# paritybit-ai/XFL

Measured on AMD Instinct MI355X. Metric: 2048-bit Paillier encrypts/s (device-resident), higher is better.
Workload: dtype u32; 1 GPU; DJN private-key (CRT) encrypt, obfuscated, precision 7, 1000000 float64 plaintexts/GPU resident in HBM; key_bits=2048, elements_per_gpu=1000000, fixed_base_window_bits=23, fixed_base_window_split=False, parallelism=shard1, table_bytes=193273528320

## Files before the change

### __graft_entry__.py

```python
import os
import sys

ROOT = os.path.dirname(os.path.abspath(__file__))
if ROOT not in sys.path:
    sys.path.insert(0, ROOT)


def build() -> None:
    from xfl_amd import build as b
    b.build()
    from oracle import build as ob
    ob.build()
    import runpy
    for script in ("build.py", "build_redc_block.py"):
        try:
            runpy.run_path(os.path.join(ROOT, "tests", "native", script), run_name="tests_native_build")["build"]()
        except Exception as exc:
            print(f"warning: device self-test harnesses not built ({script}): {exc}", file=sys.stderr)
    import xfl_amd
    from xfl_amd import _native
    _native.lib()


def smoke() -> None:
    import numpy as np

    from oracle import paillier_oracle as O
    from xfl_amd import _native as nat
    from xfl_amd.paillier.utils import getprimeover
    import random
    import math

    rng = random.Random(7)
    while True:
        p, q = getprimeover(1024, rng=rng), getprimeover(1024, rng=rng)
        if p != q and math.gcd(p - 1, q - 1) == 2:
            break
    n = p * q
    x = rng.getrandbits(n.bit_length()) | (1 << (n.bit_length() - 1))
    h = pow(-(x * x), n, n * n)
    dk = nat.DeviceKey(2048, n, p, q, h, device=0)
    ok = O.derive_private(p, q, h)
    vals = np.random.default_rng(0).standard_normal(64) * 10
    ms = [O.encode_element(ok, float(v), 7)[0] for v in vals]
    rs = [rng.randrange(1, ok["djn_exp_bound"]) for _ in vals]
    ct = nat.words_to_ints(dk.encrypt_words(nat.ints_to_words(ms, dk.nw), nat.ints_to_words(rs, dk.rand_words)))
    want = [O.encrypt_m(ok, m, r) for m, r in zip(ms, rs)]
# ... 11 lines not shown
```

### xfl_amd/csrc/bn_dev.hpp

```cpp
#pragma once
#include <hip/hip_runtime.h>
#include <stdint.h>

namespace xhe {

#define XHE_DEV __device__ __forceinline__
#define XHE_INL __attribute__((always_inline))

#ifndef XHE_SQ_ACC
#define XHE_SQ_ACC 2
#endif
XHE_DEV uint64_t mad64(uint32_t a, uint32_t b, uint64_t c) {
  asm("v_mad_u64_u32 %0, vcc, %1, %2, %0" : "+v"(c) : "v"(a), "v"(b) : "vcc");
  return c;
}
template <int N>
XHE_DEV void mad_shift(uint64_t (&T)[N], const uint32_t (&b)[N], uint32_t a) {
  int j = 1;
#pragma unroll
  for (; j + 6 <= N; j += 6)
    asm("v_mad_u64_u32 %0, vcc, %7, %8, %1\n\t"
        "v_mad_u64_u32 %1, vcc, %7, %9, %2\n\t"
        "v_mad_u64_u32 %2, vcc, %7, %10, %3\n\t"
        "v_mad_u64_u32 %3, vcc, %7, %11, %4\n\t"
// ... 473 lines not shown
    sq_columns<0, HI>(b, lo, 0ull, q, hi);
    uint64_t T[L];
#pragma unroll
    for (int j = 0; j < L; ++j) T[j] = lo[j];
    hi.sync();
    red_rows(T, hi);
    normalize(T, b);
  }
  template <class HI>
  XHE_DEV void red_rows(uint64_t (&T)[L], const HI& hi) const {
    const uint32_t* Np = np();
    NRes R;
    load_res(Np, R);
    uint64_t x0 = T[0];
    uint32_t m = ((uint32_t)x0 * n0inv) & MASK;
    uint4 cur = hi.load4(0);
    int i = 0;
    for (; i + 4 <= S; i += 4) {
      uint4 nxt = hi.load4(i + 4 < S4 ? i + 4 : i);
      __builtin_amdgcn_sched_barrier(0);
      step1_red(Np, R, T, cur.x, m, x0);
      __builtin_amdgcn_sched_barrier(0);
      step1_red(Np, R, T, cur.y, m, x0);
      __builtin_amdgcn_sched_barrier(0);
      step1_red(Np, R, T, cur.z, m, x0);
      __builtin_amdgcn_sched_barrier(0);
      step1_red(Np, R, T, cur.w, m, x0);
      __builtin_amdgcn_sched_barrier(0);
      cur = nxt;
    }
#pragma unroll
    for (int r = 0; r < (S & 3); ++r) step1_red(Np, R, T, comp4(cur, r), m, x0);
  }

  XHE_DEV void step(const uint32_t* Np, uint64_t (&T)[L], const uint32_t (&b)[L], uint32_t ai, uint32_t ai_next,
                    uint32_t& m, uint64_t& x0, bool lead) const {
    static_assert(L >= 5, "pipelined step needs L >= 5");
    uint64_t xn = 0;
    uint32_t t = 0, mn = 0;
    int stage = 0;
    auto advance = [&]() XHE_INL {
      if (stage == 0) {
        T[0] += x0 >> W;
        asm volatile("" : "+v"(T[0]));
      } else if (stage == 1) {
        xn = mad64(ai_next, b[0], T[0]);
        asm volatile("" : "+v"(xn));
      } else if (stage == 2) {
        t = (uint32_t)xn * n0inv;
        asm volatile("" : "+v"(t));
      } else if (stage == 3) {
        mn = G::bcast0(t & MASK);
        asm volatile("" : "+v"(mn));
      }
      ++stage;
      __builtin_amdgcn_sched_barrier(0);
    };
    x0 = madN(Np, m, 0, x0);
    mac4(Np, T, b, ai, m, 1);
    advance();
    int j = 5;
#pragma unroll
    for (; j + 8 <= L; j += 8) {
      mac8(Np, T, b, ai, m, j);
      if (stage < 4) advance();
    }
// ... 328 lines not shown
```

### xfl_amd/csrc/keyconst.hpp

```cpp
#pragma once
#include <algorithm>
#include <cstdint>
#include <stdexcept>
#include <utility>
#include <vector>

#include "hostbn.hpp"
#include "keydev.hpp"
#include "rns_layout.hpp"

namespace xhe {

struct ModSpec {
  int S, W;
  int S4() const { return (S + 3) & ~3; }
  BigU R() const { return pow2((size_t)W * S); }
};

struct KeySpec {
  int K;
  bool priv, djn;
  ModSpec mp2, mp2L, mp2X;
  ModSpec mp;
  ModSpec mn2, mn2X;
// ... 256 lines not shown
    }
    put(rows, {m, &ModDev::Rpow});
  }

  KeyDev bind(const uint32_t* base) const {
    KeyDev r = kd;
    for (const Binding& b : binds) {
      const uint32_t* p = base + b.off;
      if (b.dst.w) r.*b.dst.w = p;
      else if (b.dst.d) r.*b.dst.d = reinterpret_cast<const uint2*>(p);
      else (r.*b.dst.m).*b.dst.mw = p;
    }
    return r;
  }

 private:
  struct Binding {
    Dst dst;
    size_t off;
  };
  std::vector<Binding> binds;
};

namespace pq {
constexpr ModF m2[2] = {&KeyDev::p2, &KeyDev::q2}, m2L[2] = {&KeyDev::p2L, &KeyDev::q2L},
               m2X[2] = {&KeyDev::p2X, &KeyDev::q2X}, m1[2] = {&KeyDev::p, &KeyDev::q},
               dm[2] = {&KeyDev::dp, &KeyDev::dq};
constexpr RowF nprime[2] = {&KeyDev::p2_nprime, &KeyDev::q2_nprime}, rns[2] = {&KeyDev::rns_p, &KeyDev::rns_q},
               nR2[2] = {&KeyDev::nR2_p2, &KeyDev::nR2_q2}, nR2L[2] = {&KeyDev::nR2_p2L, &KeyDev::nR2_q2L},
               nR[2] = {&KeyDev::nR_p2, &KeyDev::nR_q2}, R1C[2] = {&KeyDev::R1C_p2X, &KeyDev::R1C_q2X},
               nR2C[2] = {&KeyDev::nR2C_p2X, &KeyDev::nR2C_q2X}, m1_words[2] = {&KeyDev::pm1_words, &KeyDev::qm1_words},
               inv_lim[2] = {&KeyDev::pinv_lim, &KeyDev::qinv_lim}, hR[2] = {&KeyDev::hpR, &KeyDev::hqR},
               topc[2] = {&KeyDev::topc_p, &KeyDev::topc_q}, mu[2] = {&KeyDev::mu_p, &KeyDev::mu_q},
               e_words[2] = {&KeyDev::ep_words, &KeyDev::eq_words},
               x_kn2[2] = {&KeyDev::x_kn2_p, &KeyDev::x_kn2_q}, x_rmn[2] = {&KeyDev::x_rmn_p, &KeyDev::x_rmn_q},
               x_topc[2] = {&KeyDev::x_topc_p, &KeyDev::x_topc_q}, x_fold[2] = {&KeyDev::x_fold_p, &KeyDev::x_fold_q},
               x_hpR[2] = {&KeyDev::x_hpR_p, &KeyDev::x_hpR_q};
constexpr PairF x_dwt[2] = {&KeyDev::x_dwt_p, &KeyDev::x_dwt_q}, x_dw[2] = {&KeyDev::x_dw_p, &KeyDev::x_dw_q};
constexpr IntF m1_bits[2] = {&KeyDev::pm1_bits, &KeyDev::qm1_bits}, e_bits[2] = {&KeyDev::ep_bits, &KeyDev::eq_bits};
}

struct Prime {
  BigU X, Y, X2, n, h;
};

struct DigitMod {
  const BigU& M;
  ModSpec s;
  BigU R, RM, Rinv;
  DigitMod(const BigU& M_, const ModSpec& s_) : M(M_), s(s_), R(s_.R()), RM(mod(R, M_)), Rinv(modinv(RM, M_)) {}
};

inline std::vector<uint32_t> digit_pairs(const DigitMod& d, const BigU& Xw) {
  const BigU e = mulmod(mod(Xw, d.M), d.Rinv, d.M);
  BigU Q;
  divmod(add(Xw, mul(d.R, sub(d.M, e))), d.M, &Q, nullptr);
  const BigU f = submod(mod(Q, d.M), d.RM, d.M);
  const std::vector<uint32_t> el = e.to_limbs(d.s.W, d.s.S), fl = f.to_limbs(d.s.W, d.s.S);
  std::vector<uint32_t> v(2 * (size_t)d.s.S);
  for (int i = 0; i < d.s.S; ++i) {
    v[2 * i] = el[i];
    v[2 * i + 1] = fl[i];
  }
  return v;
}

// ... 88 lines not shown
    im.put_limbs(mulmod(pr[i].n, mulmod(CR, RxP, X2), X2), sx, pq::nR2C[i]);
  }
}

inline void decrypt_constants(KeyImage& im, const KeySpec& s, const BigU& n, Prime (&pr)[2]) {
  const ModSpec& s1 = s.mp;
  const BigU T = s1.R();
  for (int i = 0; i < 2; ++i) im.put_mod(pr[i].X, s1, pq::m1[i]);
  for (int i = 0; i < 2; ++i) {
    const BigU m1 = sub(pr[i].X, BigU(1));
    im.kd.*pq::m1_bits[i] = (int)m1.bits();
    im.put_words(m1, s.nw() / 2 + 1, pq::m1_words[i]);
  }
  for (int i = 0; i < 2; ++i) im.put_limbs(modinv(pr[i].X, T), s1, pq::inv_lim[i]);
  BigU Tm[2];
  for (int i = 0; i < 2; ++i) {
    const BigU& X = pr[i].X;
    const BigU x = mod(add(BigU(1), mul(sub(X, BigU(1)), n)), pr[i].X2);
    BigU L;
    divmod(sub(x, BigU(1)), X, &L, nullptr);
    pr[i].h = modinv(L, X);
    Tm[i] = mod(T, X);
  }
  for (int i = 0; i < 2; ++i) im.put_limbs(mulmod(pr[i].h, Tm[i], pr[i].X), s1, pq::hR[i]);
  im.put_limbs(mulmod(modinv(pr[1].X, pr[0].X), Tm[0], pr[0].X), s1, &KeyDev::qinvpR);
  im.put_limbs(pr[1].X, s1, &KeyDev::q_lim);
  if (s.K == 2048)
    for (int i = 0; i < 2; ++i) im.put(mask_plus_e(pr[i].X, mod(s.pmd.R(), pr[i].X), s.pmd), pq::topc[i]);
  if (s.K == 2048 && s.djn)
    for (int i = 0; i < 2; ++i) {
      const BigU &X = pr[i].X, RX = mod(s.pmd.R(), X), R2 = mulmod(RX, RX, X);
      im.put_limbs(mulmod(mod(pr[i].Y, X), mulmod(R2, R2, X), X), s.pmd, pq::mu[i]);
    }
}

inline void pdigit_constants(KeyImage& im, const KeySpec& s, const Prime& pr, int i) {
  const BigU &X = pr.X, &X2 = pr.X2;
  const DigitMod d(X, s.pd);
  digit_modulus(im, d, X2, pq::dm[i], pq::x_kn2[i], pq::x_rmn[i]);
  im.put(mask_plus_e(X, d.RM, d.s), pq::x_topc[i]);
  im.put_limbs(mulmod(mod(pr.Y, X), mulmod(mulmod(d.RM, d.RM, X), d.RM, X), X), d.s, pq::x_fold[i]);
  const BigU Rx2 = mod(d.R, X2), R2 = mulmod(Rx2, Rx2, X2), R4 = mulmod(R2, R2, X2);
  im.put(digit_pairs(d, mulmod(R4, modinv(mod(s.mp2.R(), X2), X2), X2)), pq::x_dwt[i]);
  im.put(digit_pairs(d, R4), pq::x_dw[i]);
  im.put_limbs(mulmod(pr.h, d.RM, X), d.s, pq::x_hpR[i]);
}

inline void exponent_constants(KeyImage& im, const KeySpec& s, const BigU& n, const Prime (&pr)[2]) {
  im.put_limbs(shl(pr[0].X, 1), s.mp, &KeyDev::p2x_lim);
  im.put_limbs(pr[0].X, s.mp, &KeyDev::p_lim);
  for (int i = 0; i < 2; ++i) {
    const BigU e = mod(n, mul(pr[i].X, sub(pr[i].X, BigU(1))));
    im.kd.*pq::e_bits[i] = (int)e.bits();
    im.put_words(e, s.nw(), pq::e_words[i]);
  }
}

inline std::vector<uint32_t> inverse_base_limbs(const ModSpec& s, const BigU& h, const BigU& P) {
  std::vector<uint32_t> v = mulmod(modinv(mod(h, P), P), mod(s.R(), P), P).to_limbs(s.W, s.S);
  v.resize((size_t)s.S4(), 0u);
  return v;
}

inline KeyImage derive_key_constants(const KeySpec& s, const BigU& n, const BigU* p, const BigU* q, const BigU* h) {
  KeyImage im;
  KeyDev& kd = im.kd;
// ... 35 lines not shown
```

### xfl_amd/csrc/keydev.hpp

```cpp
#pragma once
#include <cstdint>

#include <hip/hip_vector_types.h>

namespace xhe {

struct ModDev {
  const uint32_t* N;
  const uint32_t* R1;
  const uint32_t* R2;
  const uint32_t* R3;
  uint32_t n0inv;
  const uint32_t* Rpow;
};

constexpr int kRawChunk = 32;
constexpr int kRpowRows = kRawChunk + 2;

struct KeyDev {
  int K, nw, n2w;
  int priv, djn;
  const uint32_t* n_words;
  const uint32_t* n2_words;
  const uint32_t* maxpos;
// ... 8 lines not shown
  ModDev p2, q2;
  ModDev p2L, q2L;
  ModDev p2X, q2X;
  ModDev n2X;
  const uint32_t* nR2_p2;
  const uint32_t *nR_p2, *nR_q2;
  const uint32_t *nR2C_p2X, *nR2C_q2X;
  const uint32_t *R1C_p2X, *R1C_q2X;
  const uint32_t* nR2_q2;
  const uint32_t* nR2_p2L;
  const uint32_t* nR2_q2L;
  const uint32_t* q2invR_p2;
  const uint32_t* q2_lim;
  const uint32_t* p2x4_lim;
  const uint32_t* tab_p2;
  const uint32_t* tab_q2;
  int64_t tab_rs;
  int win, nwin, nhi;
  ModDev p, q;
  const uint32_t* pm1_words;
  const uint32_t* qm1_words;
  int pm1_bits, qm1_bits;
  const uint32_t* pinv_lim;
  const uint32_t* qinv_lim;
  const uint32_t* hpR;
  const uint32_t* hqR;
  const uint32_t* qinvpR;
  const uint32_t* q_lim;
  const uint32_t* p2x_lim;
  const uint32_t* p_lim;
  int pmd;
  const uint32_t *topc_p, *topc_q;
  const uint32_t *mu_p, *mu_q;
  int ndig;
  ModDev nd;
  const uint32_t *nd_kn2, *nd_rmn, *nd_topc;
  const uint2 *nd_dw, *nd_d1;
  const uint2* nd_dwt;
  int pub_nd;
  int pmdx;
  ModDev dp, dq;
  const uint32_t *x_kn2_p, *x_kn2_q, *x_rmn_p, *x_rmn_q, *x_topc_p, *x_topc_q, *x_fold_p, *x_fold_q;
  const uint2 *x_dwt_p, *x_dwt_q;
  int pmdx_dec;
  const uint2 *x_dw_p, *x_dw_q;
  const uint32_t *x_hpR_p, *x_hpR_q;
  const uint32_t *p2_nprime, *q2_nprime;
  const uint32_t *rns, *rns_p, *rns_q;
  const uint32_t *n2w_N, *n2w_np, *n2w_C, *n2w_R2;
  const uint32_t* n2_mu;
  ModDev nL;
  const uint32_t* n2_limL;
};

}
```

### xfl_amd/csrc/pdigit_dev.hpp

```cpp
#pragma once
#include "bn_dev.hpp"

namespace xhe {

struct PmdLdsQ {
  const uint32_t* q;
  XHE_DEV uint4 load4(int i) const { return *reinterpret_cast<const uint4*>(q + (i >> 2) * 256); }
};

template <int K_>
struct PMD {
  static constexpr int K = K_, W = 28, BL = 6;
  static constexpr int NQ = (2 * K + 3) / 4;
  static constexpr uint32_t MASK = (1u << W) - 1u;
  static_assert((K - 1) % BL == 0, "positions 1..K-1 in blocks of 6");
  static_assert((double)(3 * K + 2) * (double)(1ull << 57) < 18446744073709551616.0, "accumulator bound");

  uint32_t p[K];
  uint32_t n0inv;

  XHE_DEV void init(const uint32_t* __restrict__ P, uint32_t ninv) {
#pragma unroll
    for (int j = 0; j < K; ++j) p[j] = __builtin_amdgcn_readfirstlane(P[j]);
    n0inv = ninv;
// ... 348 lines not shown
    constexpr int LQ = (LW + 3) / 4;
    constexpr int NW = HW < LW ? HW : LW;
    static_assert(HW >= 8 && HW <= 4 * LQ, "at least one block of the chain, at most a whole sum");
    uint32_t s[4 * LQ];
#pragma unroll
    for (int q = 0; q < LQ; ++q) {
      const uint4 v = *reinterpret_cast<const uint4*>(slot + (EQ + q) * 256);
      s[4 * q] = v.x, s[4 * q + 1] = v.y, s[4 * q + 2] = v.z, s[4 * q + 3] = v.w;
    }
    uint64_t cy;
    add8<true>(s, lam, 0, cy);
#pragma unroll
    for (int k = 8; k + 8 <= NW; k += 8) add8<false>(s, lam, k, cy);
#pragma unroll
    for (int k = NW & ~7; k < NW; ++k)
      asm("v_addc_co_u32_e64 %0, %1, %0, %2, %1" : "+v"(s[k]), "+s"(cy) : "v"(lam[k]));
#pragma unroll
    for (int k = NW; k < LW; ++k) asm("v_addc_co_u32_e64 %0, %1, 0, %0, %1" : "+v"(s[k]), "+s"(cy));
#pragma unroll
    for (int q = 0; q < LQ; ++q)
      *reinterpret_cast<uint4*>(slot + (EQ + q) * 256) = make_uint4(s[4 * q], s[4 * q + 1], s[4 * q + 2], s[4 * q + 3]);
  }
  XHE_DEV static void lam_add_slot(uint32_t* slot, const uint32_t* other) {
    constexpr int LQ = (LW + 3) / 4;
    uint32_t o[4 * LQ];
#pragma unroll
    for (int q = 0; q < LQ; ++q) {
      const uint4 v = *reinterpret_cast<const uint4*>(other + (EQ + q) * 256);
      o[4 * q] = v.x, o[4 * q + 1] = v.y, o[4 * q + 2] = v.z, o[4 * q + 3] = v.w;
    }
    lam_add<4 * LQ>(slot, o);
  }

  XHE_DEV void finish(const uint32_t (&a)[K], uint32_t (&c)[K], uint32_t* slot, const uint32_t* Pl) const {
    constexpr int LQ = (LW + 3) / 4;
    {
      uint32_t s[4 * LQ + 1];
#pragma unroll
      for (int q = 0; q < LQ; ++q) {
        const uint4 v = *reinterpret_cast<const uint4*>(slot + (EQ + q) * 256);
        s[4 * q] = v.x, s[4 * q + 1] = v.y, s[4 * q + 2] = v.z, s[4 * q + 3] = v.w;
      }
      s[4 * LQ] = 0u;
      auto limb = [&](int i) -> uint32_t {
        const int bit = W * i, k = bit >> 5, sh = bit & 31;
        return i < K ? (__builtin_amdgcn_alignbit(k + 1 < LW ? s[k + 1] : 0u, s[k], sh) & MASK) : 0u;
      };
#pragma unroll
      for (int q = 0; q < EQ; ++q)
        *reinterpret_cast<uint4*>(slot + q * 256) = make_uint4(limb(4 * q), limb(4 * q + 1), limb(4 * q + 2), limb(4 * q + 3));
    }
    __builtin_amdgcn_sched_barrier(0);
    uint32_t t[K];
#pragma unroll
    for (int j = 0; j < K; ++j) t[j] = a[j];
    Mont<K, W, 1> MN;
    MN.init(Pl, n0inv);
    MN.mul(t, PmdLdsQ{slot});
    uint32_t cy = 0;
#pragma unroll
    for (int j = 0; j < K; ++j) {
      const uint32_t x = c[j] + t[j] + cy;
      c[j] = j + 1 < K ? (x & MASK) : x;
      cy = j + 1 < K ? (x >> W) : 0u;
    }
  }

  XHE_DEV static void normalize(const uint64_t (&T)[K], uint32_t (&b)[K]) {
    uint64_t cy = 0;
#pragma unroll
    for (int j = 0; j < K; ++j) {
      const uint64_t x = T[j] + cy;
      b[j] = j + 1 < K ? ((uint32_t)x & MASK) : (uint32_t)x;
      cy = x >> W;
      __builtin_amdgcn_sched_barrier(0);
    }
  }

  XHE_DEV void to_mont2(const uint32_t (&a)[K], const uint32_t (&c)[K], uint32_t (&x)[2 * K]) const {
    uint64_t T[2 * K];
#pragma unroll
    for (int j = 0; j < K; ++j) {
      T[j] = 0;
      T[K + j] = a[j];
    }
#pragma unroll
    for (int i = 0; i < K; ++i) {
#pragma unroll
      for (int j = 0; j < K; ++j) T[i + j] = mad64s(c[j], p[i], T[i + j]);
    }
    uint64_t cy = 0;
#pragma unroll
    for (int j = 0; j < 2 * K; ++j) {
      const uint64_t v = T[j] + cy;
      x[j] = j + 1 < 2 * K ? ((uint32_t)v & MASK) : (uint32_t)v;
      cy = v >> W;
    }
  }
// ... 13 lines not shown
#pragma unroll
    for (int j = 1; j < K; ++j) T[i + j] = mad64s(mi, M.p[j], T[i + j]);
    __builtin_amdgcn_sched_barrier(0);
  }
#pragma unroll
  for (int j = 0; j < K; ++j) {
    const uint64_t x = T[K + j] + cy;
    t[j] = j + 1 < K ? ((uint32_t)x & MASK) : (uint32_t)x;
    cy = x >> 28;
  }
}

template <int K>
XHE_DEV void pmd_redc_words(const Mont<K, 28, 1>& MN, uint32_t* slot, const uint32_t* __restrict__ mw, int nw,
                            uint32_t (&t)[K]) {
  constexpr uint32_t MASK = PMD<K>::MASK;
  auto limb = [&](int j) -> uint32_t {
    const int bit = 28 * j, k = bit >> 5, sh = bit & 31;
    const uint32_t lo = word_or0(mw, k, nw);
    const uint32_t hi = sh + 28 > 32 ? word_or0(mw, k + 1, nw) : 0u;
    return j < 2 * K ? (uint32_t)((((uint64_t)hi << 32) | lo) >> sh) & MASK : 0u;
  };
#pragma unroll
  for (int q = 0; q < PMD<K>::EQ; ++q)
    *reinterpret_cast<uint4*>(slot + q * 256) =
        make_uint4(limb(K + 4 * q), limb(K + 4 * q + 1), limb(K + 4 * q + 2), limb(K + 4 * q + 3));
#pragma unroll
  for (int j = 0; j < K; ++j) t[j] = limb(j);
  __builtin_amdgcn_sched_barrier(0);
  MN.redc_wide(t, PmdLdsQ{slot});
}

template <int K>
XHE_DEV void pmd_lam_plain(const PMD<K>& M, uint32_t* slot, const uint32_t* __restrict__ mw, int nw,
                           const uint32_t* mu, const uint32_t* Pl) {
  using D = PMD<K>;
  constexpr int LQ = (D::LW + 3) / 4;
  Mont<K, 28, 1> MN;
  MN.init(Pl, M.n0inv);
  uint32_t t[K];
  pmd_redc_words<K>(MN, slot, mw, nw, t);
  __builtin_amdgcn_sched_barrier(0);
  MN.mul(t, ARow{mu});
  uint32_t s[4 * LQ];
#pragma unroll
  for (int k = 0; k < 4 * LQ; ++k) {
    const int bit = 32 * k, j = bit / 28, sh = bit - 28 * j;
    uint64_t v = j < K ? (uint64_t)t[j] : 0ull;
    if (j + 1 < K) v |= (uint64_t)t[j + 1] << 28;
    if (j + 2 < K) v |= (uint64_t)t[j + 2] << 56;
    s[k] = k < D::LW ? (uint32_t)(v >> sh) : 0u;
  }
#pragma unroll
  for (int q = 0; q < LQ; ++q)
    *reinterpret_cast<uint4*>(slot + (D::EQ + q) * 256) = make_uint4(s[4 * q], s[4 * q + 1], s[4 * q + 2], s[4 * q + 3]);
}

template <int K>
XHE_DEV uint32_t pmd_sub(uint32_t (&r)[K], const uint32_t (&s)[K]) {
  int64_t br = 0;
#pragma unroll
  for (int j = 0; j < K; ++j) {
    const int64_t v = (int64_t)r[j] - (int64_t)s[j] + br;
    r[j] = (uint32_t)v & ((1u << 28) - 1u);
    br = v >> 28;
  }
  return br ? 1u : 0u;
}

template <int K>
XHE_DEV bool pmd_csub(const PMD<K>& M, uint32_t (&r)[K]) {
  int64_t br = 0;
#pragma unroll
  for (int j = 0; j < K; ++j) br = ((int64_t)r[j] - (int64_t)M.p[j] + br) >> 28;
  const bool ge = br == 0;
  br = 0;
#pragma unroll
  for (int j = 0; j < K; ++j) {
    const int64_t v = (int64_t)r[j] - (int64_t)(ge ? M.p[j] : 0u) + br;
    r[j] = (uint32_t)v & ((1u << 28) - 1u);
    br = v >> 28;
  }
  return ge;
}

template <int K>
XHE_DEV void pmd_mod_small(const PMD<K>& M, uint32_t (&m)[K]) {
  constexpr uint32_t MASK = PMD<K>::MASK;
  const uint32_t mt = (m[K - 1] << 4) | (m[K - 2] >> 24);
  const uint32_t pt = (M.p[K - 1] << 4) | (M.p[K - 2] >> 24);
  const uint32_t q = mt / (pt + 1u);
  uint64_t cy = 0;
  int64_t br = 0;
#pragma unroll
  for (int j = 0; j < K; ++j) {
    const uint64_t qp = (uint64_t)q * M.p[j] + cy;
    cy = qp >> 28;
    const int64_t v = (int64_t)m[j] - (int64_t)(qp & MASK) + br;
    m[j] = (uint32_t)v & MASK;
    br = v >> 28;
  }
#pragma unroll
  for (int t = 0; t < 3; ++t) pmd_csub<K>(M, m);
}

template <int K>
XHE_DEV void pmd_from_mont2(const PMD<K>& M, const uint32_t (&X)[2 * K], const uint32_t* RmodP, uint32_t (&e)[K],
                            uint32_t (&f)[K]) {
  uint32_t m[K];
  {
    uint64_t T[2 * K];
#pragma unroll
    for (int j = 0; j < 2 * K; ++j) T[j] = X[j];
    pmd_redc_wide<K>(M, T, e, m);
  }
  __builtin_amdgcn_sched_barrier(0);
  const bool ge = pmd_csub<K>(M, e);
  __builtin_amdgcn_sched_barrier(0);
  pmd_mod_small<K>(M, m);
  __builtin_amdgcn_sched_barrier(0);
  int64_t br = 0;
#pragma unroll
  for (int j = 0; j < K; ++j) {
    const int64_t v = (int64_t)(ge ? RmodP[j] : 0u) - (int64_t)m[j] + br;
    f[j] = (uint32_t)v & ((1u << 28) - 1u);
    br = v >> 28;
  }
  if (br) {
    int64_t cy = 0;
#pragma unroll
    for (int j = 0; j < K; ++j) {
      const int64_t v = (int64_t)f[j] + (int64_t)M.p[j] + cy;
      f[j] = (uint32_t)v & ((1u << 28) - 1u);
      cy = v >> 28;
    }
  }
// ... 650 lines not shown
```

### xfl_amd/csrc/xhe.hip

```cpp
#include <hip/hip_runtime.h>
#include <stdint.h>
#include <stdlib.h>
#include <string.h>

#include <chrono>
#include <cmath>
#include <cstdio>
#include <memory>
#include <mutex>
#include <atomic>
#include <stdexcept>
#include <unordered_map>
#include <utility>
#include <string>
#include <type_traits>
#include <vector>

#include "../../include/xhe.h"
#include "abi_common.hpp"
#include "hostbn.hpp"
#include "keyconst.hpp"
#include "paths.hpp"
#include "xhe_kernels.hpp"
#include "fermat_dev.hpp"
// ... 545 lines not shown
    if (!on) return;
    if (hipEventRecord(b, s) != hipSuccess) return;
    std::lock_guard<std::mutex> lk(g_prof_mu);
    g_prof.push_back({name, a, b});
  }
};

template <class Sh, class MP2 = typename Sh::MP2>
void crt_enc_launch(const xhe_key* k, int64_t n, uint32_t* ws, uint32_t* ct, hipStream_t s) {
  const int blocks = (int)((n * MP2::TPI + 255) / 256);
  if constexpr (MP2::TPI == 1)
    launch((k_crt_enc_w<MP2, 2 * Sh::K / 32>), dim3(blocks), dim3(256), s, k->kd, k->kd.p2.N, n, ws, ct);
  else
    launch(k_crt_enc<MP2>, dim3(blocks), dim3(256), s, k->kd, k->kd.p2.N, n, ws, ct);
}

template <class Sh>
void encrypt_impl(const xhe_key* k, const uint32_t* m, const uint32_t* r, int64_t count, uint32_t* ct, hipStream_t s) {
  using MP2 = typename Sh::MP2;
  int64_t chunk = std::min<int64_t>(count, kChunk);
  WsScope wsc(s);
  uint32_t* ws = wsc.get<uint32_t>((size_t)2 * 2 * MP2::S4 * chunk * sizeof(uint32_t));
  uint2* xst = nullptr;
  uint32_t *xrows = nullptr, *xwords = nullptr;
  for (int64_t off = 0; off < count; off += chunk) {
    int64_t n = std::min(chunk, count - off);
    switch (paths::enc_djn(Sh::K, MP2::TPI, k->kd.pmd, k->kd.pmdx, n, pins())) {
      case paths::EncDjn::PMD:
        if constexpr (Sh::K == 2048) {
          ProfScope ps("k_djn_pmd", s);
          const int G = paths::pmd_split(n, pins());
          const dim3 grid((unsigned)((n * G + 127) / 128), 2);
          auto run = [&](auto kern) {
            launch(kern, grid, dim3(128), s, k->kd, k->kd.p.N, k->kd.q.N, k->kd.p2.N, k->kd.q2.N,
                   m + (size_t)off * k->nw, r + (size_t)off * k->rand_words, k->rand_words, n, ws);
          };
          if (G == 16) run(k_djn_pmd<MP2, 37, Sh::RW, 16>);
          else if (G == 4) run(k_djn_pmd<MP2, 37, Sh::RW, 4>);
          else run(k_djn_pmd<MP2, 37, Sh::RW, 1>);
          crt_enc_launch<Sh>(k, n, ws, ct + (size_t)off * k->n2w, s);
          continue;
        } else no_path("encrypt (k_djn_pmd)");
      case paths::EncDjn::PMDX:
        if constexpr (Sh::K != 2048) {
          using D = typename Sh::PDX;
          if (!xst) {
            xst = wsc.get<uint2>((size_t)2 * D::K * chunk * sizeof(uint2));
            xrows = wsc.get<uint32_t>((size_t)2 * 2 * Sh::PDXO::MN::S4 * chunk * sizeof(uint32_t));
            xwords = wsc.get<uint32_t>((size_t)2 * chunk * Sh::RW * sizeof(uint32_t));
          }
          const dim3 g4((unsigned)((n * D::TPI + 127) / 128), 2);
          {
            ProfScope ps("k_djn_pmdx", s);
            launch((k_djn_pmdx<D, Sh::RW>), g4, dim3(128), s, k->kd, r + (size_t)off * k->rand_words, k->rand_words, n,
                   xst);
          }
          using DO = typename Sh::PDXO;
          launch((k_pmdx_enc_out<DO, Sh::RW>), dim3((unsigned)((n * DO::TPI + 127) / 128), 2), dim3(128), s, k->kd,
                 m + (size_t)off * k->nw, n, xst, xrows, xwords);
          launch(k_words_to_rows<MP2>, dim3((unsigned)((n * MP2::TPI + 255) / 256), 2), dim3(256), s, xwords, Sh::RW,
                 n, ws);
          crt_enc_launch<Sh>(k, n, ws, ct + (size_t)off * k->n2w, s);
          continue;
        } else no_path("encrypt (k_djn_pmdx)");
      case paths::EncDjn::POW_X: {
        using MX = typename Sh::MP2X;
        launch((k_djn_pow_x<MX, MP2::S4, Sh::RW>), dim3((unsigned)((n * MX::TPI + 255) / 256), 2), dim3(256), s, k->kd,
// ... 1737 lines not shown
```

### xfl_amd/csrc/xhe_kernels.hpp

```cpp
#pragma once
#include "bn_dev.hpp"
#include "keydev.hpp"
#include "pdigit_dev.hpp"

#include <type_traits>

namespace xhe {

enum : int32_t { ST_OK = 0, ST_OVERFLOW = 1, ST_VALUE = 2 };

struct EncVal {
  int32_t st, e;
  int neg, w;
  uint32_t v0, v1, v2;
};

XHE_DEV EncVal encode_value(double v, int mode, int e0, int has_max, int max_exp) {
  EncVal r{ST_OK, 0, 0, 0, 0u, 0u, 0u};
  uint64_t bits = __double_as_longlong(v);
  r.neg = (int)(bits >> 63);
  int bexp = (int)((bits >> 52) & 0x7FF);
  uint64_t frac = bits & ((1ull << 52) - 1);
  int e;
  if (mode == 0) {
// ... 440 lines not shown
  }
  for (int w = 1; w < key.nwin; ++w) {
    stage(w);
    M.mul(b, ALdsQ{mine});
  }
  SqLds<MP2>(img).put(b);
  M.load_words(b, m_words + (size_t)e * key.nw, key.nw);
  M.mul(b, ARow{nR});
  b[0] += 1u;
  M.mul(b, ALdsQ{mine});
  M.reduce_once(b);
  M.store_strided(b, ws + (size_t)prime * 2 * MP2::S4 * count + e, (int)count);
}

template <class MP2, int RW>
__global__ void __launch_bounds__(128, 2) k_djn_pow_lds(KeyDev key, const uint32_t* __restrict__ Np2,
                                                        const uint32_t* __restrict__ Nq2,
                                                        const uint32_t* __restrict__ m_words,
                                                        const uint32_t* __restrict__ a_words, int aw, int64_t count,
                                                        uint32_t* __restrict__ ws) {
  static_assert(MP2::TPI == 1, "LDS row staging is per lane");
  __shared__ __attribute__((aligned(16))) uint32_t img_all[2][(MP2::S4 / 4) * 256];
  const int64_t e = (int64_t)blockIdx.x * blockDim.x + threadIdx.x;
  const int prime = blockIdx.y;
  uint32_t* img = img_all[(threadIdx.x >> 6) & 1];
  if (e >= count) return;
  djn_prime_lds<MP2, RW>(key, prime ? Nq2 : Np2, prime ? key.q2 : key.p2, prime ? key.tab_q2 : key.tab_p2,
                     prime ? key.nR2_q2 : key.nR2_p2, prime ? key.nR_q2 : key.nR_p2, m_words, a_words, aw, count, e,
                     prime, img, img + (threadIdx.x & 63) * 4, ws);
}

template <class MP2, int KP, int RW, int G = 1>
__global__ void __launch_bounds__(128, 2) k_djn_pmd(KeyDev key, const uint32_t* __restrict__ Pp,
                                                    const uint32_t* __restrict__ Pq, const uint32_t* __restrict__ Np2,
                                                    const uint32_t* __restrict__ Nq2,
                                                    const uint32_t* __restrict__ m_words,
                                                    const uint32_t* __restrict__ a_words, int aw, int64_t count,
                                                    uint32_t* __restrict__ ws) {
  static_assert(MP2::TPI == 1 && MP2::S == 2 * KP && MP2::W == 28, "digits of the one-lane P^2 shape");
  using D = PMD<KP>;
  constexpr int NQ = D::NQ > MP2::S4 / 4 ? D::NQ : MP2::S4 / 4;
  __shared__ __attribute__((aligned(16))) uint32_t img_all[2][NQ * 256];
  __shared__ __attribute__((aligned(16))) uint32_t topc[(KP + 3) & ~3];
  const int prime = blockIdx.y;
  const uint32_t* tc = prime ? key.topc_q : key.topc_p;
  if (threadIdx.x < KP) topc[threadIdx.x] = tc[threadIdx.x];
  __syncthreads();
  static_assert(G >= 1 && G <= 64 && (G & (G - 1)) == 0, "lane groups of a power of two, inside one wave");
  const int64_t t = (int64_t)blockIdx.x * blockDim.x + threadIdx.x;
  const int64_t e = t / G;
  const int g = (int)(threadIdx.x & (G - 1));
  if (e >= count) return;
  uint32_t* img = img_all[(threadIdx.x >> 6) & 1];
  uint32_t* slot = img + (threadIdx.x & 63) * 4;
  const uint32_t* tab = prime ? key.tab_q2 : key.tab_p2;
  const uint32_t* ae = a_words + (size_t)e * aw;
  D M;
  M.init(prime ? Pq : Pp, prime ? key.q.n0inv : key.p.n0inv);
  auto stage = [&](int w) XHE_INL {
    int64_t row0;
    const uint32_t d = win_digit(key, ae, aw, w, row0);
    const uint32_t* row = tab + (size_t)(row0 + d) * key.tab_rs;
#pragma unroll
    for (int k = 0; k < RW / 8; ++k)
      __builtin_amdgcn_global_load_lds((xhe_glb_void*)(row + 4 * k), (xhe_lds_void*)(img + k * 256), 16, 0, 0);
    uint32_t lam[RW / 2];
#pragma unroll
    for (int k = 0; k < RW / 8; ++k) {
      const uint4 v = *reinterpret_cast<const uint4*>(row + RW / 2 + 4 * k);
      lam[4 * k] = v.x, lam[4 * k + 1] = v.y, lam[4 * k + 2] = v.z, lam[4 * k + 3] = v.w;
    }
    asm volatile("s_waitcnt vmcnt(0)" ::: "memory");
    D::template lam_add<RW / 2>(slot, lam);
    unpack_e_lds<KP, RW / 2>(slot);
  };
  if (G == 1 || g == 0)
    pmd_lam_plain<KP>(M, slot, m_words + (size_t)e * key.nw, key.nw, prime ? key.mu_q : key.mu_p, prime ? Pq : Pp);
  else
    D::lam_zero(slot);
  __builtin_amdgcn_sched_barrier(0);
  uint32_t a[KP], c[KP];
  if (G == 1 || g < key.nwin) {
    stage(g);
#pragma unroll
    for (int q = 0; q < D::EQ; ++q) {
      const uint4 v = *reinterpret_cast<const uint4*>(slot + q * 256);
      if (4 * q < KP) a[4 * q] = v.x;
      if (4 * q + 1 < KP) a[4 * q + 1] = v.y;
      if (4 * q + 2 < KP) a[4 * q + 2] = v.z;
      if (4 * q + 3 < KP) a[4 * q + 3] = v.w;
    }
#pragma unroll
    for (int j = 0; j < KP; ++j) c[j] = 0u;
  }
  for (int w = g + G; w < key.nwin; w += G) {
    stage(w);
    M.mul_row(a, c, slot, topc);
  }
  if constexpr (G > 1) {
#pragma unroll
    for (int s = 1; s < G; s <<= 1) {
      const bool writer = (g & (2 * s - 1)) == s && g < key.nwin;
      const bool reader = (g & (2 * s - 1)) == 0 && g + s < key.nwin;
      if (reader) D::lam_add_slot(slot, slot + 4 * s);
      wave_sync_mem_();
      if (writer) {
#pragma unroll
        for (int q = 0; q < D::NQ; ++q)
          *reinterpret_cast<uint4*>(slot + q * 256) =
              make_uint4(2 * q < KP ? a[2 * q] : 0u, 2 * q < KP ? c[2 * q] : 0u, 2 * q + 1 < KP ? a[2 * q + 1] : 0u,
                         2 * q + 1 < KP ? c[2 * q + 1] : 0u);
      }
      wave_sync_mem_();
      if (reader) M.mul(a, c, slot + 4 * s, topc);
      wave_sync_mem_();
    }
    if (g != 0) return;
  }
  M.finish(a, c, slot, prime ? Pq : Pp);
  __builtin_amdgcn_sched_barrier(0);
  uint32_t b[MP2::L];
  M.to_mont2(a, c, b);
  __builtin_amdgcn_sched_barrier(0);
  MP2 N;
  N.init(prime ? Nq2 : Np2, prime ? key.q2.n0inv : key.p2.n0inv);
  N.redc_wide(b, AZero{});
  N.reduce_once(b);
  const int64_t eo = ((int64_t)blockIdx.x * blockDim.x + (uint32_t)opaque_i((int)threadIdx.x)) / G;
  N.store_strided(b, ws + (size_t)prime * 2 * MP2::S4 * count + eo, (int)count);
}

template <int KP>
XHE_DEV void pmd_pow_uniform(const PMD<KP>& M, uint32_t (&a)[KP], uint32_t (&c)[KP], const uint32_t* ex, int ebits,
                             uint4* __restrict__ tab_base, int lane, int G, uint32_t* slot, const uint32_t* topc) {
  constexpr int NQ = PMD<KP>::NQ;
#define tab (tab_base + opaque_i(lane))
  auto quad = [&](int q) -> uint4 {
    return make_uint4(2 * q < KP ? a[2 * q] : 0u, 2 * q < KP ? c[2 * q] : 0u, 2 * q + 1 < KP ? a[2 * q + 1] : 0u,
                      2 * q + 1 < KP ? c[2 * q + 1] : 0u);
  };
  auto put_slot = [&]() XHE_INL {
#pragma unroll
    for (int q = 0; q < NQ; ++q) *reinterpret_cast<uint4*>(slot + q * 256) = quad(q);
  };
  auto put_tab = [&](int t) XHE_INL {
#pragma unroll
    for (int q = 0; q < NQ; ++q) tab[((size_t)t * NQ + q) * G] = quad(q);
  };
  auto tab_to_slot = [&](int t) XHE_INL {
    uint4 v[NQ];
#pragma unroll
    for (int q = 0; q < NQ; ++q) v[q] = tab[((size_t)t * NQ + q) * G];
#pragma unroll
    for (int q = 0; q < NQ; ++q) *reinterpret_cast<uint4*>(slot + q * 256) = v[q];
  };
  auto tab_to_regs = [&](int t) XHE_INL {
#pragma unroll
    for (int q = 0; q < NQ; ++q) {
      const uint4 v = tab[((size_t)t * NQ + q) * G];
      if (2 * q < KP) a[2 * q] = v.x, c[2 * q] = v.y;
// ... 1820 lines not shown
```

Measured before the change: 50.21 million encrypts/s.

## Add short-plaintext fast path and fused PMD exit replacing mod-p² REDC

Adds a wave-uniform fast path that recognizes small-magnitude encoded plaintexts (positive or n-minus-small) and builds the lambda entry with a short 4-limb Montgomery product against a new precomputed constant, instead of a full-width word reduction. Also replaces the finish/to_mont2/redc_wide sequence at kernel exit with a fused pmd_exit that folds the top-correction subtraction into the reduction rows and directly reconstructs the mod-p² value, dropping the Np2/Nq2 arguments. The fast path only triggers when every lane in a wave has a short plaintext; otherwise it falls back to the full path. This removes per-element reduction work at both ends of the kernel but adds branching and new key constants whose correctness must match the oracle.

```diff
diff --git a/__graft_entry__.py b/__graft_entry__.py
--- a/__graft_entry__.py
+++ b/__graft_entry__.py
@@ -12,7 +12,7 @@
     from oracle import build as ob
     ob.build()
     import runpy
-    for script in ("build.py", "build_redc_block.py"):
+    for script in ("build.py", "build_redc_block.py", "build_pmd_ends.py"):
         try:
             runpy.run_path(os.path.join(ROOT, "tests", "native", script), run_name="tests_native_build")["build"]()
         except Exception as exc:
diff --git a/xfl_amd/csrc/bn_dev.hpp b/xfl_amd/csrc/bn_dev.hpp
--- a/xfl_amd/csrc/bn_dev.hpp
+++ b/xfl_amd/csrc/bn_dev.hpp
@@ -529,6 +529,41 @@
 #pragma unroll
     for (int r = 0; r < (S & 3); ++r) step1_red(Np, R, T, comp4(cur, r), m, x0);
   }
+  template <class QS>
+  XHE_DEV void red_rows_q(uint64_t (&T)[L], const QS& qs) const {
+    const uint32_t* Np = np();
+    NRes R;
+    load_res(Np, R);
+    uint64_t x0 = T[0];
+    uint32_t m = ((uint32_t)x0 * n0inv) & MASK;
+    int i = 0;
+    for (; i + 4 <= S; i += 4) {
+      uint4 d;
+      __builtin_amdgcn_sched_barrier(0);
+      d.x = m;
+      step1_red(Np, R, T, 0u, m, x0);
+      __builtin_amdgcn_sched_barrier(0);
+      d.y = m;
+      step1_red(Np, R, T, 0u, m, x0);
+      __builtin_amdgcn_sched_barrier(0);
+      d.z = m;
+      step1_red(Np, R, T, 0u, m, x0);
+      __builtin_amdgcn_sched_barrier(0);
+      d.w = m;
+      step1_red(Np, R, T, 0u, m, x0);
+      __builtin_amdgcn_sched_barrier(0);
+      qs.put4(i, d);
+    }
+    if constexpr ((S & 3) != 0) {
+      uint32_t d[4] = {0u, 0u, 0u, 0u};
+#pragma unroll
+      for (int r = 0; r < (S & 3); ++r) {
+        d[r] = m;
+        step1_red(Np, R, T, 0u, m, x0);
+      }
+      qs.put4(i, make_uint4(d[0], d[1], d[2], d[3]));
+    }
+  }
 
   XHE_DEV void step(const uint32_t* Np, uint64_t (&T)[L], const uint32_t (&b)[L], uint32_t ai, uint32_t ai_next,
                     uint32_t& m, uint64_t& x0, bool lead) const {
diff --git a/xfl_amd/csrc/keyconst.hpp b/xfl_amd/csrc/keyconst.hpp
--- a/xfl_amd/csrc/keyconst.hpp
+++ b/xfl_amd/csrc/keyconst.hpp
@@ -312,6 +312,7 @@
                nR2C[2] = {&KeyDev::nR2C_p2X, &KeyDev::nR2C_q2X}, m1_words[2] = {&KeyDev::pm1_words, &KeyDev::qm1_words},
                inv_lim[2] = {&KeyDev::pinv_lim, &KeyDev::qinv_lim}, hR[2] = {&KeyDev::hpR, &KeyDev::hqR},
                topc[2] = {&KeyDev::topc_p, &KeyDev::topc_q}, mu[2] = {&KeyDev::mu_p, &KeyDev::mu_q},
+               ms[2] = {&KeyDev::ms_p, &KeyDev::ms_q},
                e_words[2] = {&KeyDev::ep_words, &KeyDev::eq_words},
                x_kn2[2] = {&KeyDev::x_kn2_p, &KeyDev::x_kn2_q}, x_rmn[2] = {&KeyDev::x_rmn_p, &KeyDev::x_rmn_q},
                x_topc[2] = {&KeyDev::x_topc_p, &KeyDev::x_topc_q}, x_fold[2] = {&KeyDev::x_fold_p, &KeyDev::x_fold_q},
@@ -466,6 +467,11 @@
       const BigU &X = pr[i].X, RX = mod(s.pmd.R(), X), R2 = mulmod(RX, RX, X);
       im.put_limbs(mulmod(mod(pr[i].Y, X), mulmod(R2, R2, X), X), s.pmd, pq::mu[i]);
     }
+  if (s.K == 2048 && s.djn)
+    for (int i = 0; i < 2; ++i) {
+      const BigU &X = pr[i].X, RX = mod(s.pmd.R(), X), R2 = mulmod(RX, RX, X);
+      im.put_limbs(mulmod(mulmod(mod(pr[i].Y, X), R2, X), mod(pow2((size_t)s.pmd.W * 4), X), X), s.pmd, pq::ms[i]);
+    }
 }
 
 inline void pdigit_constants(KeyImage& im, const KeySpec& s, const Prime& pr, int i) {
diff --git a/xfl_amd/csrc/keydev.hpp b/xfl_amd/csrc/keydev.hpp
--- a/xfl_amd/csrc/keydev.hpp
+++ b/xfl_amd/csrc/keydev.hpp
@@ -64,6 +64,7 @@
   int pmd;
   const uint32_t *topc_p, *topc_q;
   const uint32_t *mu_p, *mu_q;
+  const uint32_t *ms_p, *ms_q;
   int ndig;
   ModDev nd;
   const uint32_t *nd_kn2, *nd_rmn, *nd_topc;
diff --git a/xfl_amd/csrc/pdigit_dev.hpp b/xfl_amd/csrc/pdigit_dev.hpp
--- a/xfl_amd/csrc/pdigit_dev.hpp
+++ b/xfl_amd/csrc/pdigit_dev.hpp
@@ -404,38 +404,22 @@
     lam_add<4 * LQ>(slot, o);
   }
 
-  XHE_DEV void finish(const uint32_t (&a)[K], uint32_t (&c)[K], uint32_t* slot, const uint32_t* Pl) const {
+  XHE_DEV static void lam_to_limbs(uint32_t* slot) {
     constexpr int LQ = (LW + 3) / 4;
-    {
-      uint32_t s[4 * LQ + 1];
-#pragma unroll
-      for (int q = 0; q < LQ; ++q) {
-        const uint4 v = *reinterpret_cast<const uint4*>(slot + (EQ + q) * 256);
-        s[4 * q] = v.x, s[4 * q + 1] = v.y, s[4 * q + 2] = v.z, s[4 * q + 3] = v.w;
-      }
-      s[4 * LQ] = 0u;
-      auto limb = [&](int i) -> uint32_t {
-        const int bit = W * i, k = bit >> 5, sh = bit & 31;
-        return i < K ? (__builtin_amdgcn_alignbit(k + 1 < LW ? s[k + 1] : 0u, s[k], sh) & MASK) : 0u;
-      };
-#pragma unroll
-      for (int q = 0; q < EQ; ++q)
-        *reinterpret_cast<uint4*>(slot + q * 256) = make_uint4(limb(4 * q), limb(4 * q + 1), limb(4 * q + 2), limb(4 * q + 3));
-    }
-    __builtin_amdgcn_sched_barrier(0);
-    uint32_t t[K];
-#pragma unroll
-    for (int j = 0; j < K; ++j) t[j] = a[j];
-    Mont<K, W, 1> MN;
-    MN.init(Pl, n0inv);
-    MN.mul(t, PmdLdsQ{slot});
-    uint32_t cy = 0;
-#pragma unroll
-    for (int j = 0; j < K; ++j) {
-      const uint32_t x = c[j] + t[j] + cy;
-      c[j] = j + 1 < K ? (x & MASK) : x;
-      cy = j + 1 < K ? (x >> W) : 0u;
-    }
+    uint32_t s[4 * LQ + 1];
+#pragma unroll
+    for (int q = 0; q < LQ; ++q) {
+      const uint4 v = *reinterpret_cast<const uint4*>(slot + (EQ + q) * 256);
+      s[4 * q] = v.x, s[4 * q + 1] = v.y, s[4 * q + 2] = v.z, s[4 * q + 3] = v.w;
+    }
+    s[4 * LQ] = 0u;
+    auto limb = [&](int i) -> uint32_t {
+      const int bit = W * i, k = bit >> 5, sh = bit & 31;
+      return i < K ? (__builtin_amdgcn_alignbit(k + 1 < LW ? s[k + 1] : 0u, s[k], sh) & MASK) : 0u;
+    };
+#pragma unroll
+    for (int q = 0; q < EQ; ++q)
+      *reinterpret_cast<uint4*>(slot + q * 256) = make_uint4(limb(4 * q), limb(4 * q + 1), limb(4 * q + 2), limb(4 * q + 3));
   }
 
   XHE_DEV static void normalize(const uint64_t (&T)[K], uint32_t (&b)[K]) {
@@ -515,28 +499,102 @@
 }
 
 template <int K>
+XHE_DEV void pmd_lam_store(uint32_t* slot, const uint32_t (&t)[K]) {
+  using D = PMD<K>;
+  constexpr int LQ = (D::LW + 3) / 4;
+  uint32_t s[4 * LQ];
+#pragma unroll
+  for (int k = 0; k < 4 * LQ; ++k) {
+    const int bit = 32 * k, j = bit / 28, sh = bit - 28 * j;
+    uint64_t v = j < K ? (uint64_t)t[j] : 0ull;
+    if (j + 1 < K) v |= (uint64_t)t[j + 1] << 28;
+    if (j + 2 < K) v |= (uint64_t)t[j + 2] << 56;
+    s[k] = k < D::LW ? (uint32_t)(v >> sh) : 0u;
+  }
+#pragma unroll
+  for (int q = 0; q < LQ; ++q)
+    *reinterpret_cast<uint4*>(slot + (D::EQ + q) * 256) = make_uint4(s[4 * q], s[4 * q + 1], s[4 * q + 2], s[4 * q + 3]);
+}
+
+template <int K>
 XHE_DEV void pmd_lam_plain(const PMD<K>& M, uint32_t* slot, const uint32_t* __restrict__ mw, int nw,
                            const uint32_t* mu, const uint32_t* Pl) {
-  using D = PMD<K>;
-  constexpr int LQ = (D::LW + 3) / 4;
   Mont<K, 28, 1> MN;
   MN.init(Pl, M.n0inv);
   uint32_t t[K];
   pmd_redc_words<K>(MN, slot, mw, nw, t);
   __builtin_amdgcn_sched_barrier(0);
   MN.mul(t, ARow{mu});
-  uint32_t s[4 * LQ];
-#pragma unroll
-  for (int k = 0; k < 4 * LQ; ++k) {
-    const int bit = 32 * k, j = bit / 28, sh = bit - 28 * j;
-    uint64_t v = j < K ? (uint64_t)t[j] : 0ull;
-    if (j + 1 < K) v |= (uint64_t)t[j + 1] << 28;
-    if (j + 2 < K) v |= (uint64_t)t[j + 2] << 56;
-    s[k] = k < D::LW ? (uint32_t)(v >> sh) : 0u;
-  }
-#pragma unroll
-  for (int q = 0; q < LQ; ++q)
-    *reinterpret_cast<uint4*>(slot + (D::EQ + q) * 256) = make_uint4(s[4 * q], s[4 * q + 1], s[4 * q + 2], s[4 * q + 3]);
+  pmd_lam_store<K>(slot, t);
+}
+
+constexpr int kPmdShortLimbs = 4;
+template <int K>
+XHE_DEV bool pmd_short_classify(const uint32_t* __restrict__ mw, int nw, const uint32_t* __restrict__ nwords,
+                                uint32_t (&s)[4], bool& neg) {
+  constexpr int MW = (28 * 2 * K) / 32;
+  static_assert(kPmdShortLimbs * 28 > 96 && kPmdShortLimbs * 28 <= 128, "the magnitude ends in the fourth word");
+  constexpr uint32_t TOP = 1u << (kPmdShortLimbs * 28 - 96);
+  uint32_t lo[4], d[4], hz = 0u, hd = 0u, br = 0u;
+#pragma unroll
+  for (int k = 0; k < MW; ++k) {
+    const uint32_t m = word_or0(mw, k, nw), n = word_or0(nwords, k, nw);
+    const uint64_t x = (uint64_t)n - (uint64_t)m - (uint64_t)br;
+    br = (uint32_t)(x >> 63);
+    if (k < 4) {
+      lo[k] = m;
+      d[k] = (uint32_t)x;
+    } else {
+      hz |= m;
+      hd |= (uint32_t)x;
+    }
+  }
+  const bool pos = hz == 0u && lo[3] < TOP;
+  neg = !pos && br == 0u && hd == 0u && d[3] < TOP && (d[0] | d[1] | d[2] | d[3]) != 0u;
+#pragma unroll
+  for (int k = 0; k < 4; ++k) s[k] = pos ? lo[k] : d[k];
+  return pos || neg;
+}
+
+template <int K>
+XHE_DEV void pmd_lam_short(const PMD<K>& M, uint32_t* slot, const uint32_t (&sw)[4], bool neg,
+                           const uint32_t* __restrict__ ms) {
+  constexpr int L = kPmdShortLimbs;
+  constexpr uint32_t MASK = PMD<K>::MASK;
+  const uint32_t sl[L] = {sw[0] & MASK, ((sw[0] >> 28) | (sw[1] << 4)) & MASK, ((sw[1] >> 24) | (sw[2] << 8)) & MASK,
+                          ((sw[2] >> 20) | (sw[3] << 12)) & MASK};
+  uint64_t T[K + L];
+#pragma unroll
+  for (int j = 0; j < K + L; ++j) T[j] = 0;
+#pragma unroll
+  for (int j = 0; j < K; ++j) {
+    const uint32_t mj = ms[j];
+#pragma unroll
+    for (int i = 0; i < L; ++i) T[i + j] = mad64s(sl[i], mj, T[i + j]);
+  }
+#pragma unroll
+  for (int i = 0; i < L; ++i) {
+    const uint32_t q = ((uint32_t)T[i] * M.n0inv) & MASK;
+#pragma unroll
+    for (int j = 0; j < K; ++j) T[i + j] = mad64s(q, M.p[j], T[i + j]);
+    T[i + 1] += T[i] >> 28;
+  }
+  uint32_t v[K];
+  uint64_t cy = 0;
+#pragma unroll
+  for (int j = 0; j < K; ++j) {
+    const uint64_t x = T[L + j] + cy;
+    v[j] = (uint32_t)x & MASK;
+    cy = x >> 28;
+  }
+  int64_t br = 0;
+#pragma unroll
+  for (int j = 0; j < K; ++j) {
+    const int64_t x = (int64_t)(2u * M.p[j]) - (int64_t)v[j] + br;
+    v[j] = neg ? ((uint32_t)x & MASK) : v[j];
+    br = x >> 28;
+  }
+  pmd_lam_store<K>(slot, v);
 }
 
 template <int K>
@@ -585,6 +643,92 @@
   }
 #pragma unroll
   for (int t = 0; t < 3; ++t) pmd_csub<K>(M, m);
+}
+
+struct PmdTopcSink {
+  uint32_t* slot;
+  const uint32_t* topc;
+  XHE_DEV void put4(int i, const uint4& m) const {
+    const uint4 tc = *reinterpret_cast<const uint4*>(topc + i);
+    *reinterpret_cast<uint4*>(slot + (i >> 2) * 256) = make_uint4(tc.x - m.x, tc.y - m.y, tc.z - m.z, tc.w - m.w);
+  }
+};
+
+template <int K>
+XHE_DEV void pmd_exit(const PMD<K>& M, const uint32_t (&a)[K], const uint32_t (&c)[K], uint32_t* slot,
+                      const uint32_t* topc, const uint32_t* Pl, uint32_t (&x)[2 * K]) {
+  using D = PMD<K>;
+  constexpr uint32_t MASK = D::MASK;
+  Mont<K, 28, 1> MN;
+  MN.init(Pl, M.n0inv);
+  uint32_t u[K], z[K];
+  {
+    uint64_t T[K];
+#pragma unroll
+    for (int j = 0; j < K; ++j) T[j] = a[j];
+    MN.red_rows_q(T, PmdTopcSink{slot, topc});
+    MN.normalize(T, u);
+  }
+  __builtin_amdgcn_sched_barrier(0);
+  {
+    uint32_t wv[K];
+#pragma unroll
+    for (int q = 0; q < D::EQ; ++q) {
+      const uint4 v = *reinterpret_cast<const uint4*>(slot + q * 256);
+      if (4 * q < K) wv[4 * q] = v.x;
+      if (4 * q + 1 < K) wv[4 * q + 1] = v.y;
+      if (4 * q + 2 < K) wv[4 * q + 2] = v.z;
+      if (4 * q + 3 < K) wv[4 * q + 3] = v.w;
+    }
+    __builtin_amdgcn_sched_barrier(0);
+    D::lam_to_limbs(slot);
+    __builtin_amdgcn_sched_barrier(0);
+    uint64_t T[K];
+#pragma unroll
+    for (int j = 0; j < K; ++j) T[j] = c[j];
+    MN.run(T, u, PmdLdsQ{slot});
+    MN.normalize(T, z);
+    uint32_t cy = 0;
+#pragma unroll
+    for (int j = 0; j < K; ++j) {
+      const uint32_t v = z[j] + wv[j] + cy;
+      T[j] = j + 1 < K ? (v & MASK) : v;
+      cy = v >> 28;
+    }
+    __builtin_amdgcn_sched_barrier(0);
+    MN.red_rows(T, AZero{});
+    MN.normalize(T, z);
+  }
+  __builtin_amdgcn_sched_barrier(0);
+  pmd_csub<K>(M, z);
+  const bool up = pmd_csub<K>(M, u);
+  uint32_t cy = up ? 1u : 0u;
+#pragma unroll
+  for (int j = 0; j < K; ++j) {
+    const uint32_t v = z[j] + cy;
+    z[j] = v & MASK;
+    cy = v >> 28;
+  }
+  pmd_csub<K>(M, z);
+  __builtin_amdgcn_sched_barrier(0);
+  uint64_t T[2 * K];
+#pragma unroll
+  for (int j = 0; j < K; ++j) {
+    T[j] = u[j];
+    T[K + j] = 0;
+  }
+#pragma unroll
+  for (int i = 0; i < K; ++i) {
+#pragma unroll
+    for (int j = 0; j < K; ++j) T[i + j] = mad64s(z[j], M.p[i], T[i + j]);
+  }
+  uint64_t c2 = 0;
+#pragma unroll
+  for (int j = 0; j < 2 * K; ++j) {
+    const uint64_t v = T[j] + c2;
+    x[j] = (uint32_t)v & MASK;
+    c2 = v >> 28;
+  }
 }
 
 template <int K>
diff --git a/xfl_amd/csrc/xhe.hip b/xfl_amd/csrc/xhe.hip
--- a/xfl_amd/csrc/xhe.hip
+++ b/xfl_amd/csrc/xhe.hip
@@ -601,7 +601,7 @@
           const int G = paths::pmd_split(n, pins());
           const dim3 grid((unsigned)((n * G + 127) / 128), 2);
           auto run = [&](auto kern) {
-            launch(kern, grid, dim3(128), s, k->kd, k->kd.p.N, k->kd.q.N, k->kd.p2.N, k->kd.q2.N,
+            launch(kern, grid, dim3(128), s, k->kd, k->kd.p.N, k->kd.q.N,
                    m + (size_t)off * k->nw, r + (size_t)off * k->rand_words, k->rand_words, n, ws);
           };
           if (G == 16) run(k_djn_pmd<MP2, 37, Sh::RW, 16>);
diff --git a/xfl_amd/csrc/xhe_kernels.hpp b/xfl_amd/csrc/xhe_kernels.hpp
--- a/xfl_amd/csrc/xhe_kernels.hpp
+++ b/xfl_amd/csrc/xhe_kernels.hpp
@@ -496,8 +496,7 @@
 
 template <class MP2, int KP, int RW, int G = 1>
 __global__ void __launch_bounds__(128, 2) k_djn_pmd(KeyDev key, const uint32_t* __restrict__ Pp,
-                                                    const uint32_t* __restrict__ Pq, const uint32_t* __restrict__ Np2,
-                                                    const uint32_t* __restrict__ Nq2,
+                                                    const uint32_t* __restrict__ Pq,
                                                     const uint32_t* __restrict__ m_words,
                                                     const uint32_t* __restrict__ a_words, int aw, int64_t count,
                                                     uint32_t* __restrict__ ws) {
@@ -538,10 +537,18 @@
     D::template lam_add<RW / 2>(slot, lam);
     unpack_e_lds<KP, RW / 2>(slot);
   };
-  if (G == 1 || g == 0)
-    pmd_lam_plain<KP>(M, slot, m_words + (size_t)e * key.nw, key.nw, prime ? key.mu_q : key.mu_p, prime ? Pq : Pp);
-  else
+  if (G == 1 || g == 0) {
+    const uint32_t* mw = m_words + (size_t)e * key.nw;
+    uint32_t sw[4];
+    bool neg;
+    const bool is_short = pmd_short_classify<KP>(mw, key.nw, key.n_words, sw, neg);
+    if (__builtin_amdgcn_ballot_w64(!is_short) == 0ull)
+      pmd_lam_short<KP>(M, slot, sw, neg, prime ? key.ms_q : key.ms_p);
+    else
+      pmd_lam_plain<KP>(M, slot, mw, key.nw, prime ? key.mu_q : key.mu_p, prime ? Pq : Pp);
+  } else {
     D::lam_zero(slot);
+  }
   __builtin_amdgcn_sched_barrier(0);
   uint32_t a[KP], c[KP];
   if (G == 1 || g < key.nwin) {
@@ -581,15 +588,10 @@
     }
     if (g != 0) return;
   }
-  M.finish(a, c, slot, prime ? Pq : Pp);
-  __builtin_amdgcn_sched_barrier(0);
   uint32_t b[MP2::L];
-  M.to_mont2(a, c, b);
+  pmd_exit<KP>(M, a, c, slot, topc, prime ? Pq : Pp, b);
   __builtin_amdgcn_sched_barrier(0);
   MP2 N;
-  N.init(prime ? Nq2 : Np2, prime ? key.q2.n0inv : key.p2.n0inv);
-  N.redc_wide(b, AZero{});
-  N.reduce_once(b);
   const int64_t eo = ((int64_t)blockIdx.x * blockDim.x + (uint32_t)opaque_i((int)threadIdx.x)) / G;
   N.store_strided(b, ws + (size_t)prime * 2 * MP2::S4 * count + eo, (int)count);
 }
```

New measurement: 50.86 million encrypts/s (median of 6 runs). 1.3% higher.
